# OpenDriveLab/OccNet

Hardware: AMD Instinct MI355X
Metric: nuScenes samples/sec (6-cam 900x1600 -> 200x200x16 voxels) (higher is better)
Workload: dtype f32 hot path (GEMM operands bf16x3-split, SCA value rows q16 block floating point) + bf16 backbone; 1 GPU; bevformer_base_occ forward: 6x(3x928x1600) images -> ResNet-50+FPN -> 4 BEVFormer layers (TSA+SCA+FFN) -> lifter + 2xConv3d decoder -> 200x200x16 voxels x (17 logits + 2 flow); history_frames=0, mode=infer, scope=e2e, input=resident-f32, samples_per_gpu=1, global_batch=1, parallelism=dp1, step_graph=False, linear_precision=bf16x3, backbone_dtype=bf16

## Files before the change

### include/occnet_amd.h

```cpp
#ifndef OCCNET_AMD_H_
#define OCCNET_AMD_H_

#include <stdint.h>

#ifdef __cplusplus
extern "C" {
#endif

#define OCC_OK 0
#define OCC_E_INVALID (-1)
#define OCC_E_LAUNCH (-2)
#define OCC_E_UNSUPPORTED (-3)

int occ_abi_version(void);
const char* occ_last_error(void);
int occ_selftest_fdiv_f32(const float* a, const float* d, float* q, int64_t n, void* stream);


int occ_ms_deform_attn_forward_f32(const float* value, const int64_t* spatial_shapes,
                                   const int64_t* level_start_index, const float* sampling_loc,
                                   const float* attn_weight, float* out, int B, int S, int M, int D,
                                   int L, int Lq, int P, int im2col_step, void* stream);

int occ_ms_deform_attn_backward_f32(const float* value, const int64_t* spatial_shapes,
// ... 120 lines not shown
                                     float* zv, int64_t ldzv, int M, void* stream);

int occ_sca_prep_forward_f32(const float* proj, int64_t proj_batch_stride, int proj_ld, const int64_t* row_to_query,
                             const float* ref_rb, const int64_t* spatial_shapes, float* loc, float* attn, int B,
                             int64_t R, int M, int L, int P, int Z, void* stream);
int occ_sca_prep_backward_f32(const float* grad_loc, const float* grad_attn, const float* attn,
                              const int64_t* query_to_rows, int Kq, const int64_t* spatial_shapes, float* dproj,
                              int proj_ld, int B, int64_t R, int64_t Q, int M, int L, int P, void* stream);

int occ_rows_gather_sum_f32(const float* x, int64_t x_batch_stride, const int64_t* index, int K, float* out, int B,
                            int64_t rows_out, int64_t rows_in, int F, void* stream);

int64_t occ_linear_wgrad_workspace_bytes(int M, int N, int K);
int occ_linear_wgrad_bf16x3_f32(const float* dy, int64_t lddy, const float* x, int64_t ldx, float* dw, float* db,
                                void* workspace, int64_t workspace_bytes, int M, int N, int K, void* stream);

int64_t occ_conv3d_wgrad_workspace_bytes(int B, int Z, int Y, int X, int Cin);
int occ_conv3d_wgrad_bf16x3_f32(const float* dy_pad, const float* x_pad, float* dw, void* workspace,
                                int64_t workspace_bytes, int B, int Z, int Y, int X, int Cin, void* stream);

int occ_bias_act_nhwc_bf16(void* x, const float* bias, const void* residual, int64_t rows, int C, int relu,
                           void* stream);

int64_t occ_bias_act_bwd_partial_floats(int64_t rows, int C);
int occ_bias_act_bwd_nhwc_bf16(const void* grad_y, const void* y, void* g, float* partial, float* bias_grad,
                               int64_t rows, int C, int relu, void* stream);

int occ_conv_bn_fold_fwd_f32(const float* weight, const float* gamma, const float* beta, const float* rstd,
                             const float* mean_rstd, float* w_folded, void* w_folded_bf16_nhwc, float* bias, int Cout,
                             int Cin, int KH, int KW, void* stream);
int occ_conv_bn_fold_bwd_f32(const void* grad_w_bf16, int64_t stride_o, int64_t stride_i, int64_t stride_h, int64_t stride_w,
                             const float* weight, const float* gamma, const float* rstd, const float* mean_rstd,
                             const float* grad_bias, float* grad_weight, float* grad_gamma, int Cout, int Cin, int KH, int KW,
                             void* stream);

unsigned occ_ln_dropout_hash(unsigned index, unsigned seed_lo, unsigned seed_hi);
int64_t occ_dropout_add_ln_bwd_partial_floats(int64_t rows, int C);
int occ_dropout_add_ln_fwd_f32(const float* x, const float* residual, const float* gamma, const float* beta, float eps,
                               float p_drop, uint64_t seed, float* z, float* y, float* stats, int64_t rows, int C,
                               void* stream);
int occ_dropout_add_ln_bwd_f32(const float* grad_y, const float* z, const float* stats, const float* gamma, float p_drop,
                               uint64_t seed, float* grad_x, float* grad_residual, float* partial, float* grad_gamma_beta,
                               int64_t rows, int C, void* stream);

int occ_value_proj_bf16_f32(int n_segments, const void* const* a, const int64_t* lda, const int64_t* rows,
                            const int64_t* rows_per_group, const int64_t* out_row0,
                            const float* const* group_bias, int bias_groups, const void* weight_packed,
                            float* out, int64_t ldo, int K, int N, int64_t out_group_rows, void* stream);
int occ_value_proj_bf16_f16pairs(int n_segments, const void* const* a, const int64_t* lda, const int64_t* rows,
                            const int64_t* rows_per_group, const int64_t* out_row0,
                            const float* const* group_bias, int bias_groups, const void* weight_packed,
                            void* out, int64_t ldo, int K, int N, int64_t out_group_rows, const float* out_scale,
                            void* stream);
int occ_value_proj_bf16_q16pairs(int n_segments, const void* const* a, const int64_t* lda, const int64_t* rows,
                            const int64_t* rows_per_group, const int64_t* out_row0,
                            const float* const* group_bias, int bias_groups, const void* weight_packed,
                            void* out, int64_t ldo, int K, int N, int64_t out_group_rows, const float* out_scale,
                            void* stream);

int occ_value_range_scale_bf16(int n_segments, const void* const* a, const int64_t* lda, const int64_t* rows, int K,
                               int n_planes, const float* row_l1, const float* bias_max, float* scale_out,
                               uint32_t* work, void* stream);
int occ_value_range_scale_from_amax(const uint32_t* amax8, int n_planes, const float* row_l1, const float* bias_max,
                                    float* scale_out, void* stream);

int occ_value_proj_bf16_planes(int n_segments, const void* const* a, const int64_t* lda, const int64_t* rows,
                               const int64_t* rows_per_group, const int64_t* out_row0,
                               const float* const* group_bias, int bias_groups, const void* weight_packed, void* out,
                               int out_f16, int64_t ldo, int K, int n_planes, int plane_cols, int64_t plane_stride,
                               int64_t out_group_rows, const float* out_scale, void* stream);

int occ_stem_conv7x7_pool_f32_bf16(const float* x, const void* weight_frag, const float* bias, void* out,
                                   int batch, int H, int W, void* stream);
int occ_stem_conv7x7_pool_u8_bf16(const uint8_t* x, const void* weight_frag, const float* bias, void* out,
                                  int batch, int Hs, int Ws, int H, int W, const float* mean,
                                  const float* std, int to_rgb, void* stream);

int occ_bias_relu_maxpool_nhwc_bf16(const void* y, const float* bias, void* out, int batch, int H, int W, int C,
                                    void* stream);

int occ_conv1x1_nhwc_bf16(const void* x, const void* weight, const float* bias, const void* residual,
                          void* out, int batch, int Hin, int Win, int Cin, int Cout, int stride, int relu,
                          int residual_upsample2, void* stream);

int occ_conv3x3_pack_weight_bf16(const float* weight, void* packed, int Cout, int Cin, void* stream);
int occ_conv3x3_nhwc_bf16(const void* x, const void* weight_packed, const float* bias, void* out, int batch,
                          int H, int W, int Cin, int Cout, int stride, int relu, void* stream);
int occ_conv3x3_nhwc_bf16_amax(const void* x, const void* weight_packed, const float* bias, void* out, int batch,
                               int H, int W, int Cin, int Cout, int stride, int relu, uint32_t* amax8, void* stream);
int occ_conv3x3_nhwc_bf16_variant(const void* x, const void* weight_packed, const float* bias, void* out, int batch,
                                  int H, int W, int Cin, int Cout, int stride, int relu, uint32_t* amax8, int variant,
                                  void* stream);

int occ_mfma_pack_b_frag_bf16(const float* weight, void* packed, int N, int K, void* stream);

int occ_bottleneck64_nhwc_bf16(const void* x, const void* w1_frag, const float* b1, const void* w2_frag,
                               const float* b2, const void* w3_frag, const float* b3, void* out, int batch,
                               int H, int W, int Cin, int downsample, void* stream);

#ifdef __cplusplus
}
#endif
#endif
```

### occnet_amd/csrc/conv1x1_nhwc_bf16.hip

```cpp
#include "common.h"

namespace occ {

typedef float f32x16 __attribute__((ext_vector_type(16)));
typedef __bf16 bf16x8 __attribute__((ext_vector_type(8)));


__device__ __forceinline__ float c1_bf16_to_f32(unsigned short h) { return __uint_as_float((unsigned)h << 16); }

template <int NT, int RT>
__global__ __launch_bounds__(256) void conv1x1_nhwc_bf16_kernel(
    const uint4* __restrict__ x, const uint4* __restrict__ w, const float* __restrict__ bias,
    const unsigned short* __restrict__ residual, unsigned short* __restrict__ out, long M, int N, int K,
    int Hin, int Win, int Hout, int Wout, int stride, int relu, int res_up) {
  constexpr int KC = 32, kCLD = KC * 2 + 16, PC = KC / 8;
  constexpr int BM = 32 * RT, BN = 128 * NT, WR = 32 * NT, OLD = BN + 4;
  constexpr int AP = BM * PC / 256;
  constexpr int A_BYTES = BM * kCLD;
  constexpr int STAGE_BYTES = 2 * A_BYTES, OUT_BYTES = 32 * OLD * 4;
  __shared__ __attribute__((aligned(16))) char lds[STAGE_BYTES > OUT_BYTES ? STAGE_BYTES : OUT_BYTES];
  const int tid = threadIdx.x, lane = tid & 63, wave = tid >> 6;
  const int vi = lane & 31, kb = lane >> 5;
  const long m0 = (long)blockIdx.x * BM;
  const int n0 = blockIdx.y * BN;
  const int KQ = K / 8;
  const int NT32 = N / 32;

  f32x16 acc[RT][NT];
#pragma unroll
  for (int rt = 0; rt < RT; ++rt)
#pragma unroll
    for (int t = 0; t < NT; ++t)
#pragma unroll
      for (int r = 0; r < 16; ++r) acc[rt][t][r] = 0.f;

  static_assert(AP >= 1 && AP <= 2 && NT <= 2, "staging register budget");
  long aofs[AP];
  int adst[AP];
#pragma unroll
  for (int ap = 0; ap < AP; ++ap) {
    const int j = tid + 256 * ap;
    const int row = j / PC, piece = j % PC;
    long m = m0 + row;
    if (m >= M) m = M - 1;
    long pix = m;
    if (stride != 1) {
      const long hw = (long)Hout * Wout;
      const long n = m / hw, rem = m % hw;
      const int yo = (int)(rem / Wout), xo = (int)(rem % Wout);
      pix = (n * Hin + (long)yo * stride) * Win + (long)xo * stride;
    }
    aofs[ap] = pix * KQ + piece;
    adst[ap] = row * kCLD + piece * 16;
  }
  const int nt0 = min((n0 + wave * WR) / 32, NT32 - 1), nt1 = min((n0 + wave * WR) / 32 + (NT - 1), NT32 - 1);
  const long wl0 = (long)nt0 * 64 + lane, wl1 = (long)nt1 * 64 + lane;
  uint4 va0_0, va1_0, va0_1, va1_1;
  uint4 wa0_0, wa1_0, wb0_0, wb1_0, wa0_1, wa1_1, wb0_1, wb1_1, wa0_2, wa1_2, wb0_2, wb1_2;
#define OCC_C1_ISSUE_A(S, K0)                                                                     \
  {                                                                                               \
    const long kq = (K0) / 8;                                                                     \
    va0_##S = x[aofs[0] + kq];                                                                    \
    if (AP > 1) va1_##S = x[aofs[AP > 1 ? 1 : 0] + kq];                                           \
  }
#define OCC_C1_ISSUE_W(S, K0)                                                                     \
  {                                                                                               \
    const long k0 = (long)((K0) / 16) * NT32 * 64, k1 = k0 + (long)NT32 * 64;                     \
    wa0_##S = w[k0 + wl0]; wb0_##S = w[k1 + wl0];                                                 \
    if (NT > 1) { wa1_##S = w[k0 + wl1]; wb1_##S = w[k1 + wl1]; }                                 \
  }
#define OCC_C1_STEP(SA, SW, SWN, BUF, K_NEXT)                                                     \
  {                                                                                               \
    char* sA = lds + (BUF) * A_BYTES;                                                             \
    *reinterpret_cast<uint4*>(sA + adst[0]) = va0_##SA;                                           \
    if (AP > 1) *reinterpret_cast<uint4*>(sA + adst[AP > 1 ? 1 : 0]) = va1_##SA;                  \
    __syncthreads();                 \
    OCC_C1_ISSUE_A(SA, K_NEXT)                                                                    \
    OCC_C1_ISSUE_W(SWN, K_NEXT)                                                                   \
    bf16x8 af[RT][2];                                                                             \
    _Pragma("unroll") for (int rt = 0; rt < RT; ++rt)                                             \
      _Pragma("unroll") for (int ks = 0; ks < 2; ++ks)                                            \
        af[rt][ks] = *reinterpret_cast<const bf16x8*>(sA + (rt * 32 + vi) * kCLD + ks * 32 + kb * 16); \
    _Pragma("unroll") for (int rt = 0; rt < RT; ++rt) {                                           \
      acc[rt][0] = __builtin_amdgcn_mfma_f32_32x32x16_bf16(af[rt][0], __builtin_bit_cast(bf16x8, wa0_##SW), acc[rt][0], 0, 0, 0); \
      if (NT > 1) acc[rt][NT - 1] = __builtin_amdgcn_mfma_f32_32x32x16_bf16(af[rt][0], __builtin_bit_cast(bf16x8, wa1_##SW), acc[rt][NT - 1], 0, 0, 0); \
    }                                                                                             \
    _Pragma("unroll") for (int rt = 0; rt < RT; ++rt) {                                           \
      acc[rt][0] = __builtin_amdgcn_mfma_f32_32x32x16_bf16(af[rt][1], __builtin_bit_cast(bf16x8, wb0_##SW), acc[rt][0], 0, 0, 0); \
      if (NT > 1) acc[rt][NT - 1] = __builtin_amdgcn_mfma_f32_32x32x16_bf16(af[rt][1], __builtin_bit_cast(bf16x8, wb1_##SW), acc[rt][NT - 1], 0, 0, 0); \
    }                                                                                             \
  }

  const int NCHK = K / KC;
  const int rot = (int)((blockIdx.x * 5u + blockIdx.y * 3u) % (unsigned)NCHK);
#define OCC_C1_K(CI) ((((CI) < NCHK ? (CI) : NCHK - 1) + rot) % NCHK * KC)
  OCC_C1_ISSUE_A(0, OCC_C1_K(0))
  OCC_C1_ISSUE_W(0, OCC_C1_K(0))
  OCC_C1_ISSUE_A(1, OCC_C1_K(1))
  OCC_C1_ISSUE_W(1, OCC_C1_K(1))
  for (int ci = 0; ci < NCHK; ci += 6) {
    OCC_C1_STEP(0, 0, 2, 0, OCC_C1_K(ci + 2))
    if (ci + 1 < NCHK) OCC_C1_STEP(1, 1, 0, 1, OCC_C1_K(ci + 3))
    if (ci + 2 < NCHK) OCC_C1_STEP(0, 2, 1, 0, OCC_C1_K(ci + 4))
    if (ci + 3 < NCHK) OCC_C1_STEP(1, 0, 2, 1, OCC_C1_K(ci + 5))
    if (ci + 4 < NCHK) OCC_C1_STEP(0, 1, 0, 0, OCC_C1_K(ci + 6))
    if (ci + 5 < NCHK) OCC_C1_STEP(1, 2, 1, 1, OCC_C1_K(ci + 7))
  }
#undef OCC_C1_K
#undef OCC_C1_STEP
#undef OCC_C1_ISSUE_A
#undef OCC_C1_ISSUE_W

  const int c = lane * 4;
  const bool col_live = c < BN && n0 + c < N;
  float4 bv = make_float4(0.f, 0.f, 0.f, 0.f);
  if (col_live) bv = *reinterpret_cast<const float4*>(bias + n0 + c);
  float* sO = reinterpret_cast<float*>(lds);
#pragma unroll
  for (int rt = 0; rt < RT; ++rt) {
    __syncthreads();
#pragma unroll
    for (int t = 0; t < NT; ++t)
#pragma unroll
      for (int r = 0; r < 16; ++r)
        sO[((r & 3) + 8 * (r >> 2) + 4 * kb) * OLD + (wave * NT + t) * 32 + vi] = acc[rt][t][r];
    __syncthreads();
    uint2 rv[8];
#pragma unroll
    for (int rr = 0; rr < 8; ++rr) {
      long m = m0 + rt * 32 + wave * 8 + rr;
      if (m >= M) m = M - 1;
      rv[rr] = make_uint2(0u, 0u);
      if (residual != nullptr && col_live) {
        long rrow = m;
        if (res_up) {
          const long hw = (long)Hout * Wout;
          const long n = m / hw, rem = m - n * hw;
          const int yo = (int)(rem / Wout), xo = (int)(rem - (long)yo * Wout);
          rrow = (n * (Hout >> 1) + (yo >> 1)) * (Wout >> 1) + (xo >> 1);
        }
        rv[rr] = *reinterpret_cast<const uint2*>(residual + rrow * N + n0 + c);
      }
    }
#pragma unroll
    for (int rr = 0; rr < 8; ++rr) {
      const int row = wave * 8 + rr;
      const long m = m0 + rt * 32 + row;
      if (m < M && col_live) {
        float4 v = *reinterpret_cast<const float4*>(sO + row * OLD + c);
        v.x += bv.x; v.y += bv.y; v.z += bv.z; v.w += bv.w;
        v.x += c1_bf16_to_f32((unsigned short)(rv[rr].x & 0xffffu));
        v.y += c1_bf16_to_f32((unsigned short)(rv[rr].x >> 16));
        v.z += c1_bf16_to_f32((unsigned short)(rv[rr].y & 0xffffu));
        v.w += c1_bf16_to_f32((unsigned short)(rv[rr].y >> 16));
        if (relu) {
          v.x = fmaxf(v.x, 0.f); v.y = fmaxf(v.y, 0.f); v.z = fmaxf(v.z, 0.f); v.w = fmaxf(v.w, 0.f);
        }
        const uint2 o = make_uint2(pack_bf16x2_rne(v.x, v.y), pack_bf16x2_rne(v.z, v.w));
        *reinterpret_cast<uint2*>(out + m * N + n0 + c) = o;
      }
    }
  }
}

}

extern "C" int occ_conv1x1_nhwc_bf16(const void* x, const void* weight, const float* bias,
                                     const void* residual, void* out, int batch, int Hin, int Win,
                                     int Cin, int Cout, int stride, int relu, int residual_upsample2,
                                     void* stream) {
  using namespace occ;
  OCC_CHECK_ARG(x && weight && bias && out, "conv1x1_nhwc_bf16: null pointer argument");
  OCC_CHECK_ARG(batch > 0 && Hin > 0 && Win > 0 && Cin > 0 && Cout > 0 && stride > 0,
                "conv1x1_nhwc_bf16: bad dimension");
  if (Cin % 32 || Cout % 32) {
    set_error("conv1x1_nhwc_bf16: no kernel for Cin=%d Cout=%d (need Cin %% 32 == 0, Cout %% 32 == 0)", Cin,
              Cout);
    return OCC_E_UNSUPPORTED;
  }
  const int Hout = (Hin - 1) / stride + 1, Wout = (Win - 1) / stride + 1;
  OCC_CHECK_ARG(!residual_upsample2 || (residual && Hout % 2 == 0 && Wout % 2 == 0),
                "conv1x1_nhwc_bf16: an upsampled residual needs even output sizes (exact x2 nearest upsampling)");
  const long M = (long)batch * Hout * Wout;
  hipStream_t st = reinterpret_cast<hipStream_t>(stream);
#define OCC_C1_LAUNCH(NTT, RTT, BNN)                                                                \
  hipLaunchKernelGGL((conv1x1_nhwc_bf16_kernel<NTT, RTT>),                                          \
                     dim3((unsigned)((M + 32 * RTT - 1) / (32 * RTT)), (unsigned)((Cout + BNN - 1) / BNN)), \
                     dim3(256), 0, st, reinterpret_cast<const uint4*>(x),                           \
                     reinterpret_cast<const uint4*>(weight), bias,                                  \
                     reinterpret_cast<const unsigned short*>(residual),                             \
                     reinterpret_cast<unsigned short*>(out), M, Cout, Cin, Hin, Win, Hout, Wout, stride, relu,  \
                     residual_upsample2)
  if (Cout <= 128) OCC_C1_LAUNCH(1, 2, 128); else OCC_C1_LAUNCH(2, 2, 256);
#undef OCC_C1_LAUNCH
  OCC_CHECK_LAUNCH("conv1x1_nhwc_bf16");
  return OCC_OK;
}
```

### occnet_amd/ext.py

```python
import ctypes
import os

import torch

from . import _lib, cache_epoch
from ._lib import OccAmdError, OccAmdUnsupported, f32, i32, i64, ptr, stream_ptr


_TIMING = None
_TIMING_ONLY = None


def kernel_timing(enable=True):
    global _TIMING, _TIMING_ONLY
    _TIMING = {} if enable else None
    _TIMING_ONLY = None
    return _TIMING


def kernel_timing_only(names):
    global _TIMING_ONLY
    _TIMING_ONLY = None if names is None else set(names)


# ... 1330 lines not shown
    so, si, sh, sw = grad_w16.stride()
    with torch.cuda.device(weight.device):
        rc = _lib.lib().occ_conv_bn_fold_bwd_f32(ptr(grad_w16), i64(so), i64(si), i64(sh), i64(sw), ptr(weight), ptr(gamma),
                                                 ptr(rstd), ptr(mean_rstd), ptr(grad_bias), ptr(dW), ptr(dgamma), i32(O), i32(I),
                                                 i32(KH), i32(KW), stream_ptr(weight.device))
    _lib.check(rc, "conv_bn_fold_bwd")
    return dW, dgamma


def stem_pack_weight(weight):
    if tuple(weight.shape) != (64, 3, 7, 7):
        raise OccAmdUnsupported("stem_pack_weight: expected a (64, 3, 7, 7) weight")
    w2 = torch.zeros(64, 7, 8, 4, dtype=torch.float32, device=weight.device)
    w2[:, :, :7, :3] = weight.float().permute(0, 2, 3, 1)
    return mfma_pack_b_frag(w2.reshape(64, 224))


def stem_conv7x7_pool(x, weight_frag, bias):
    _need_cuda_f32("x", x)
    _need_cuda_f32("bias", bias)
    if x.dim() != 4 or x.shape[1] != 3 or not x.is_contiguous():
        raise OccAmdUnsupported("stem_conv7x7_pool: x must be a contiguous (N, 3, H, W) fp32 tensor")
    if weight_frag.numel() != 64 * 224 or bias.numel() != 64:
        raise OccAmdError("stem_conv7x7_pool: inconsistent shapes")
    N, _, H, W = x.shape
    Hc, Wc = (H - 1) // 2 + 1, (W - 1) // 2 + 1
    Hp, Wp = (Hc - 1) // 2 + 1, (Wc - 1) // 2 + 1
    out = torch.empty((N, 64, Hp, Wp), dtype=torch.bfloat16, device=x.device, memory_format=torch.channels_last)
    with torch.cuda.device(x.device), _timed('bb_stem7x7_pool'):
        rc = _lib.lib().occ_stem_conv7x7_pool_f32_bf16(ptr(x), ptr(weight_frag), ptr(bias), ptr(out), i32(N),
                                                       i32(H), i32(W), stream_ptr(x.device))
    _note_flops('bb_stem7x7_pool', 2.0 * N * Hc * Wc * 64 * 147)
    _lib.check(rc, "stem_conv7x7_pool")
    return out


def stem_conv7x7_pool_u8(x_u8, weight_frag, bias, mean, std, to_rgb=False, size_divisor=32):
    if not (x_u8.is_cuda and x_u8.dtype == torch.uint8 and x_u8.dim() == 4 and x_u8.shape[-1] == 3
            and x_u8.is_contiguous()):
        raise OccAmdUnsupported("stem_conv7x7_pool_u8: x must be a contiguous (N, H, W, 3) uint8 device tensor")
    _need_cuda_f32("bias", bias)
    if weight_frag.numel() != 64 * 224 or bias.numel() != 64:
        raise OccAmdError("stem_conv7x7_pool_u8: inconsistent shapes")
    N, Hs, Ws, _ = x_u8.shape
    d = int(size_divisor)
    H, W = (Hs + d - 1) // d * d, (Ws + d - 1) // d * d
    Hc, Wc = (H - 1) // 2 + 1, (W - 1) // 2 + 1
    Hp, Wp = (Hc - 1) // 2 + 1, (Wc - 1) // 2 + 1
    out = torch.empty((N, 64, Hp, Wp), dtype=torch.bfloat16, device=x_u8.device, memory_format=torch.channels_last)
    mean_c = (f32 * 3)(*[float(v) for v in mean])
    std_c = (f32 * 3)(*[float(v) for v in std])
    with torch.cuda.device(x_u8.device):
        rc = _lib.lib().occ_stem_conv7x7_pool_u8_bf16(ptr(x_u8), ptr(weight_frag), ptr(bias), ptr(out), i32(N),
                                                      i32(Hs), i32(Ws), i32(H), i32(W), mean_c, std_c,
                                                      i32(1 if to_rgb else 0), stream_ptr(x_u8.device))
    _lib.check(rc, "stem_conv7x7_pool_u8")
    return out, (H, W)


def bias_relu_maxpool_nhwc(y, bias):
    if not (y.is_cuda and y.dtype == torch.bfloat16 and y.dim() == 4
            and y.is_contiguous(memory_format=torch.channels_last)):
        raise OccAmdUnsupported("bias_relu_maxpool_nhwc: y must be a channels_last bfloat16 device tensor")
    _need_cuda_f32("bias", bias)
    N, C, H, W = y.shape
    if bias.numel() != C:
        raise OccAmdError("bias_relu_maxpool_nhwc: bias must have C entries")
    out = torch.empty((N, C, (H - 1) // 2 + 1, (W - 1) // 2 + 1), dtype=torch.bfloat16, device=y.device,
                      memory_format=torch.channels_last)
    with torch.cuda.device(y.device):
        rc = _lib.lib().occ_bias_relu_maxpool_nhwc_bf16(ptr(y), ptr(bias), ptr(out), i32(N), i32(H), i32(W),
                                                        i32(C), stream_ptr(y.device))
    _lib.check(rc, "bias_relu_maxpool_nhwc")
    return out


def conv1x1_pack_weight(weight2d):
    cout, cin = weight2d.shape
    if cin % 32 or cout % 32:
        raise OccAmdUnsupported("conv1x1_pack_weight: Cin and Cout must be multiples of 32")
    return mfma_pack_b_frag(weight2d.float().contiguous())


def conv1x1_nhwc(x, weight_frag, bias, residual=None, relu=False, stride=1, residual_upsample2=False):
    if not (x.is_cuda and x.dtype == torch.bfloat16 and x.dim() == 4
            and x.is_contiguous(memory_format=torch.channels_last)):
        raise OccAmdUnsupported("conv1x1_nhwc: x must be a channels_last bfloat16 device tensor")
    _need_cuda_f32("bias", bias)
    N, Cin, H, W = x.shape
    Cout = bias.numel()
    if not (weight_frag.dtype == torch.int16 and weight_frag.dim() == 1 and weight_frag.is_contiguous()
            and weight_frag.numel() == Cout * Cin):
        raise OccAmdError("conv1x1_nhwc: weight must come from conv1x1_pack_weight (Cout*Cin bf16, fragment order)")
    s = int(stride)
    Ho, Wo = (H - 1) // s + 1, (W - 1) // s + 1
    out = torch.empty((N, Cout, Ho, Wo), dtype=torch.bfloat16, device=x.device,
                      memory_format=torch.channels_last)
    want = (N, Cout, Ho // 2, Wo // 2) if residual_upsample2 else tuple(out.shape)
    if residual_upsample2 and (residual is None or Ho % 2 or Wo % 2):
        raise OccAmdUnsupported("conv1x1_nhwc: an upsampled residual needs even output sizes")
    if residual is not None and not (residual.dtype == torch.bfloat16 and tuple(residual.shape) == want and
                                     residual.is_contiguous(memory_format=torch.channels_last)):
        raise OccAmdUnsupported("conv1x1_nhwc: residual must match the output (channels_last bfloat16)")
    with torch.cuda.device(x.device), _timed('bb_conv1x1'):
        rc = _lib.lib().occ_conv1x1_nhwc_bf16(ptr(x), ptr(weight_frag), ptr(bias), ptr(residual), ptr(out),
                                              i32(N), i32(H), i32(W), i32(Cin), i32(Cout), i32(s),
                                              i32(1 if relu else 0), i32(1 if residual_upsample2 else 0),
                                              stream_ptr(x.device))
    _note_flops('bb_conv1x1', 2.0 * N * Ho * Wo * Cin * Cout)
    _lib.check(rc, "conv1x1_nhwc")
    return out


def mfma_pack_b_frag(weight2d):
    _need_cuda_f32("weight", weight2d)
    if weight2d.dim() != 2:
        raise OccAmdError("mfma_pack_b_frag: expected a (N, K) matrix")
    weight2d = weight2d.contiguous()
    n, k = weight2d.shape
    packed = torch.empty(n * k, dtype=torch.int16, device=weight2d.device)
    with torch.cuda.device(weight2d.device):
        rc = _lib.lib().occ_mfma_pack_b_frag_bf16(ptr(weight2d), ptr(packed), i32(n), i32(k),
                                                  stream_ptr(weight2d.device))
    _lib.check(rc, "mfma_pack_b_frag")
    return packed


def bottleneck64_pack(w1, b1, w2, b2, w3, b3, wds=None, bds=None):
    w1 = w1.float().reshape(w1.shape[0], -1)
    w3 = w3.float().reshape(w3.shape[0], -1)
    if tuple(w2.shape) != (64, 64, 3, 3) or w1.shape[0] != 64 or tuple(w3.shape) != (256, 64):
        raise OccAmdUnsupported("bottleneck64_pack: only 64 mid / 256 output channels")
    ds = wds is not None
    cin = w1.shape[1]
    if (ds and cin != 64) or (not ds and cin != 256):
        raise OccAmdUnsupported("bottleneck64_pack: Cin must be 256 (identity) or 64 (projection)")
    w2m = w2.float().permute(0, 2, 3, 1).reshape(64, 9 * 64)
    b3 = b3.float()
    if ds:
        w3 = torch.cat([w3, wds.float().reshape(256, 64)], dim=1)
        b3 = b3 + bds.float()
    return dict(w1=mfma_pack_b_frag(w1), b1=b1.float().contiguous(), w2=mfma_pack_b_frag(w2m),
                b2=b2.float().contiguous(), w3=mfma_pack_b_frag(w3), b3=b3.contiguous(), cin=cin, ds=ds)


def bottleneck64_nhwc(x, pack):
    if not (x.is_cuda and x.dtype == torch.bfloat16 and x.dim() == 4
            and x.is_contiguous(memory_format=torch.channels_last)):
        raise OccAmdUnsupported("bottleneck64_nhwc: x must be a channels_last bfloat16 device tensor")
    N, Cin, H, W = x.shape
    if Cin != pack['cin']:
        raise OccAmdError("bottleneck64_nhwc: x has %d channels, the pack was built for %d" % (Cin, pack['cin']))
    out = torch.empty((N, 256, H, W), dtype=torch.bfloat16, device=x.device, memory_format=torch.channels_last)
    with torch.cuda.device(x.device), _timed('bb_bottleneck64'):
        rc = _lib.lib().occ_bottleneck64_nhwc_bf16(ptr(x), ptr(pack['w1']), ptr(pack['b1']), ptr(pack['w2']),
                                                   ptr(pack['b2']), ptr(pack['w3']), ptr(pack['b3']), ptr(out),
                                                   i32(N), i32(H), i32(W), i32(Cin), i32(1 if pack['ds'] else 0),
                                                   stream_ptr(x.device))
    _note_flops('bb_bottleneck64', 2.0 * N * H * W * (Cin * 64 + 9 * 64 * 64 + 64 * 256 + (Cin * 256 if pack['ds'] else 0)))
    _lib.check(rc, "bottleneck64_nhwc")
    return out


def conv3x3_pack_weight(weight):
    _need_cuda_f32("weight", weight)
    if weight.dim() != 4 or tuple(weight.shape[2:]) != (3, 3):
        raise OccAmdError("conv3x3_pack_weight: expected a (Cout, Cin, 3, 3) weight")
    cout, cin = weight.shape[:2]
    packed = torch.empty(weight.numel(), dtype=torch.int16, device=weight.device)
    with torch.cuda.device(weight.device):
        rc = _lib.lib().occ_conv3x3_pack_weight_bf16(ptr(weight), ptr(packed), i32(cout), i32(cin),
                                                     stream_ptr(weight.device))
    _lib.check(rc, "conv3x3_pack_weight")
    return packed


def conv3x3_nhwc(x, w_packed, bias, cout, relu=False, stride=1, amax=None, variant=None):
    if not (x.is_cuda and x.dtype == torch.bfloat16 and x.dim() == 4
            and x.is_contiguous(memory_format=torch.channels_last)):
        raise OccAmdUnsupported("conv3x3_nhwc: x must be a channels_last bfloat16 device tensor")
    _need_cuda_f32("bias", bias)
    N, Cin, H, W = x.shape
    if w_packed.numel() != cout * Cin * 9 or bias.numel() != cout:
        raise OccAmdError("conv3x3_nhwc: inconsistent shapes")
    st = int(stride)
    if st not in (1, 2):
        raise OccAmdUnsupported("conv3x3_nhwc: stride must be 1 or 2")
    if amax is not None and not (amax.is_cuda and amax.dtype == torch.int32 and amax.numel() == 8 and amax.is_contiguous()):
        raise OccAmdError("conv3x3_nhwc: amax must be 8 contiguous int32 device words")
    out = torch.empty((N, cout, (H - 1) // st + 1, (W - 1) // st + 1), dtype=torch.bfloat16, device=x.device,
                      memory_format=torch.channels_last)
# ... 18 lines not shown
```

### tools_dev/conv_probe.py

```python
import os, sys
sys.path.insert(0, os.path.join(os.path.dirname(os.path.abspath(__file__)), ".."))
import torch
from occnet_amd import ext


def timeit(fn, iters=20):
    for _ in range(3):
        fn()
    a, b = torch.cuda.Event(enable_timing=True), torch.cuda.Event(enable_timing=True)
    torch.cuda.synchronize(); a.record()
    for _ in range(iters):
        fn()
    b.record(); torch.cuda.synchronize()
    return a.elapsed_time(b) * 1e3 / iters


def main(which):
    g = torch.Generator().manual_seed(0)
    N = 6
    mk = lambda *s: (torch.randn(*s, generator=g) * 0.05).cuda()
    act = lambda c, h, w: torch.randn(N, c, h, w, generator=g).cuda().to(torch.bfloat16).contiguous(
        memory_format=torch.channels_last)
    if 'c3' in which or 'c3v' in which:
        def variants(s, cout):
            if 'c3v' not in which:
                return (None,)
            vs = (12, 13, 14, 16, 18, 22, 23, 24) if s == 1 else (12, 13, 22)
            return (None,) + tuple(v for v in vs if cout % (128 * (v // 10)) == 0)
        for (cin, cout, h, w, s) in [(128, 128, 232, 400, 2), (128, 128, 116, 200, 1), (256, 256, 116, 200, 2),
                                     (256, 256, 58, 100, 1), (512, 512, 58, 100, 2), (512, 512, 29, 50, 1),
                                     (256, 256, 116, 200, 1), (256, 256, 29, 50, 1),
                                     (256, 256, 29, 50, 2)]:
            x, wp, b = act(cin, h, w), ext.conv3x3_pack_weight(mk(cout, cin, 3, 3)), mk(cout)
            vs = variants(s, cout)
            rounds = 5 if len(vs) > 1 else 1
            times = {v: [] for v in vs}
            for _ in range(rounds):
                for v in vs:
                    times[v].append(timeit(lambda: ext.conv3x3_nhwc(x, wp, b, cout, relu=True, stride=s, variant=v)))
            for v in vs:
                us = sorted(times[v])[rounds // 2]
                ho, wo = (h - 1) // s + 1, (w - 1) // s + 1
                fl = 2.0 * N * ho * wo * cout * cin * 9
                tag = 'auto' if v is None else f'v{v}'
                print(f"conv3x3 {cin:4d}->{cout:4d} {h:3d}x{w:3d} s{s} {tag:4s}: {us:7.1f} us  {fl / us * 1e-6:6.1f} TF/s")
    if 'c1' in which:
        for (cin, cout, h, w, s, res) in [(256, 128, 232, 400, 1, 0), (128, 512, 116, 200, 1, 1),
                                          (512, 128, 116, 200, 1, 0), (256, 512, 232, 400, 2, 0),
                                          (512, 256, 116, 200, 1, 0), (256, 1024, 58, 100, 1, 1),
                                          (1024, 256, 58, 100, 1, 0), (512, 1024, 116, 200, 2, 0),
                                          (1024, 512, 58, 100, 1, 0), (512, 2048, 29, 50, 1, 1),
                                          (2048, 512, 29, 50, 1, 0), (1024, 2048, 58, 100, 2, 0),
                                          (512, 256, 116, 200, 1, 0), (1024, 256, 58, 100, 1, 0),
                                          (2048, 256, 29, 50, 1, 0)]:
            x, wp, b = act(cin, h, w), ext.conv1x1_pack_weight(mk(cout, cin)), mk(cout)
            ho, wo = (h - 1) // s + 1, (w - 1) // s + 1
            r = act(cout, ho, wo) if res else None
            us = timeit(lambda: ext.conv1x1_nhwc(x, wp, b, residual=r, relu=True, stride=s))
            fl = 2.0 * N * ho * wo * cout * cin
            mb = N * (ho * wo * (cin + cout * (2 if res else 1))) * 2 / 1e6
            print(f"conv1x1 {cin:4d}->{cout:4d} {h:3d}x{w:3d} s{s} res{res}: {us:7.1f} us  {fl / us * 1e-6:6.1f} TF/s  "
                  f"{mb / us:5.2f} TB/s")


def vp():
    g = torch.Generator().manual_seed(0)
    w = (torch.randn(256, 256, generator=g) / 16).cuda()
    gb = torch.randn(6, 256, generator=g).cuda()
    total = 23200 + 5800 + 1450 + 375
    out = torch.empty(6 * total, 256, device='cuda')
    hws = (23200, 5800, 1450, 375)
    a_list = [torch.randn(6 * hw, 256, generator=g).cuda().to(torch.bfloat16) for hw in hws]
    gb4 = gb.unsqueeze(0).repeat(4, 1, 1).contiguous()
    starts = [0, 23200, 29000, 30450]
    us = timeit(lambda: ext.value_proj_bf16(a_list, w, gb4, out, rows_per_group=list(hws), out_group_rows=total,
                                            out_row0=starts))
    mb = 6 * total * 256 * (2 + 4) / 1e6
    print(f"value_proj_bf16 all levels M={6 * total}: {us:7.1f} us  {mb / us:5.2f} TB/s")
    x = torch.randn(6 * total, 256, generator=g).cuda()
    b = torch.randn(256, generator=g).cuda()
    us = timeit(lambda: ext.linear(x, w, b))
    print(f"linear bf16x3 f32 in M={6 * total}: {us:7.1f} us")


if __name__ == '__main__':
    if 'vp' in sys.argv[1:]:
        vp()
    main(sys.argv[1:] or ['c3', 'c1'])
```

Baseline: 190.2 samples/s.

## Add split-K and tile-size variants to conv1x1 NHWC kernel with per-shape pick table

```diff
diff --git a/include/occnet_amd.h b/include/occnet_amd.h
--- a/include/occnet_amd.h
+++ b/include/occnet_amd.h
@@ -226,6 +226,11 @@
 int occ_conv1x1_nhwc_bf16(const void* x, const void* weight, const float* bias, const void* residual,
                           void* out, int batch, int Hin, int Win, int Cin, int Cout, int stride, int relu,
                           int residual_upsample2, void* stream);
+int occ_conv1x1_nhwc_bf16_variant(const void* x, const void* weight, const float* bias, const void* residual,
+                                  void* out, int batch, int Hin, int Win, int Cin, int Cout, int stride, int relu,
+                                  int residual_upsample2, int variant, void* workspace, int64_t workspace_bytes,
+                                  void* stream);
+int64_t occ_conv1x1_nhwc_bf16_workspace_bytes(int batch, int Hin, int Win, int Cin, int Cout, int stride, int variant);
 
 int occ_conv3x3_pack_weight_bf16(const float* weight, void* packed, int Cout, int Cin, void* stream);
 int occ_conv3x3_nhwc_bf16(const void* x, const void* weight_packed, const float* bias, void* out, int batch,
diff --git a/occnet_amd/csrc/conv1x1_nhwc_bf16.hip b/occnet_amd/csrc/conv1x1_nhwc_bf16.hip
--- a/occnet_amd/csrc/conv1x1_nhwc_bf16.hip
+++ b/occnet_amd/csrc/conv1x1_nhwc_bf16.hip
@@ -12,7 +12,8 @@
 __global__ __launch_bounds__(256) void conv1x1_nhwc_bf16_kernel(
     const uint4* __restrict__ x, const uint4* __restrict__ w, const float* __restrict__ bias,
     const unsigned short* __restrict__ residual, unsigned short* __restrict__ out, long M, int N, int K,
-    int Hin, int Win, int Hout, int Wout, int stride, int relu, int res_up) {
+    int Hin, int Win, int Hout, int Wout, int stride, int relu, int res_up, float* __restrict__ slabs,
+    unsigned* __restrict__ tile_cnt) {
   constexpr int KC = 32, kCLD = KC * 2 + 16, PC = KC / 8;
   constexpr int BM = 32 * RT, BN = 128 * NT, WR = 32 * NT, OLD = BN + 4;
   constexpr int AP = BM * PC / 256;
@@ -91,9 +92,11 @@
     }                                                                                             \
   }
 
-  const int NCHK = K / KC;
+  const int nslice = (int)gridDim.z, slice = (int)blockIdx.z;
+  const int c_lo = (int)((long)slice * (K / KC) / nslice);
+  const int NCHK = (int)((long)(slice + 1) * (K / KC) / nslice) - c_lo;
   const int rot = (int)((blockIdx.x * 5u + blockIdx.y * 3u) % (unsigned)NCHK);
-#define OCC_C1_K(CI) ((((CI) < NCHK ? (CI) : NCHK - 1) + rot) % NCHK * KC)
+#define OCC_C1_K(CI) (((((CI) < NCHK ? (CI) : NCHK - 1) + rot) % NCHK + c_lo) * KC)
   OCC_C1_ISSUE_A(0, OCC_C1_K(0))
   OCC_C1_ISSUE_W(0, OCC_C1_K(0))
   OCC_C1_ISSUE_A(1, OCC_C1_K(1))
@@ -110,6 +113,53 @@
 #undef OCC_C1_STEP
 #undef OCC_C1_ISSUE_A
 #undef OCC_C1_ISSUE_W
+
+  if (nslice > 1) {
+    constexpr int TILE_G = BM * BN / 2;
+    const long tile = (long)blockIdx.y * gridDim.x + blockIdx.x;
+    unsigned long long* tslab = reinterpret_cast<unsigned long long*>(slabs) + tile * nslice * TILE_G;
+#pragma unroll
+    for (int rt = 0; rt < RT; ++rt)
+#pragma unroll
+      for (int t = 0; t < NT; ++t)
+#pragma unroll
+        for (int q = 0; q < 8; ++q) {
+          const unsigned long long g = ((unsigned long long)__float_as_uint(acc[rt][t][2 * q + 1]) << 32) |
+                                       __float_as_uint(acc[rt][t][2 * q]);
+          __hip_atomic_store(tslab + (long)slice * TILE_G + (((rt * NT + t) * 4 + wave) * 8 + q) * 64 + lane, g,
+                             __ATOMIC_RELAXED, __HIP_MEMORY_SCOPE_AGENT);
+        }
+    asm volatile("s_waitcnt vmcnt(0)" ::: "memory");
+    __syncthreads();
+    int* last_flag = reinterpret_cast<int*>(lds);
+    if (tid == 0) {
+      const unsigned prev = __hip_atomic_fetch_add(tile_cnt + tile, 1u, __ATOMIC_RELAXED, __HIP_MEMORY_SCOPE_AGENT);
+      *last_flag = prev == (unsigned)(nslice - 1);
+    }
+    __syncthreads();
+    if (!*last_flag) return;
+#pragma unroll
+    for (int rt = 0; rt < RT; ++rt)
+#pragma unroll
+      for (int t = 0; t < NT; ++t) {
+        f32x16 sum;
+        for (int sl = 0; sl < nslice; ++sl) {
+          f32x16 v = acc[rt][t];
+          if (sl != slice) {
+            unsigned long long* src = tslab + (long)sl * TILE_G + (((rt * NT + t) * 4 + wave) * 8) * 64 + lane;
+#pragma unroll
+            for (int q = 0; q < 8; ++q) {
+              const unsigned long long g = __hip_atomic_load(src + q * 64, __ATOMIC_RELAXED, __HIP_MEMORY_SCOPE_AGENT);
+              v[2 * q] = __uint_as_float((unsigned)g);
+              v[2 * q + 1] = __uint_as_float((unsigned)(g >> 32));
+            }
+          }
+          if (sl == 0) sum = v;
+          else sum += v;
+        }
+        acc[rt][t] = sum;
+      }
+  }
 
   const int c = lane * 4;
   const bool col_live = c < BN && n0 + c < N;
@@ -163,12 +213,41 @@
   }
 }
 
-}
-
-extern "C" int occ_conv1x1_nhwc_bf16(const void* x, const void* weight, const float* bias,
-                                     const void* residual, void* out, int batch, int Hin, int Win,
-                                     int Cin, int Cout, int stride, int relu, int residual_upsample2,
-                                     void* stream) {
+
+__global__ __launch_bounds__(256) void conv1x1_clear_counters_kernel(unsigned* __restrict__ cnt, int n) {
+  for (int i = blockIdx.x * 256 + threadIdx.x; i < n; i += gridDim.x * 256)
+    __hip_atomic_store(cnt + i, 0u, __ATOMIC_RELAXED, __HIP_MEMORY_SCOPE_AGENT);
+}
+
+bool c1_variant_known(int id) {
+  const int s = id / 100, nt = id / 10 % 10, rt = id % 10;
+  return id > 0 && (s == 0 || s == 2 || s == 4 || s == 8) && (nt == 1 || nt == 2) && (rt == 2 || rt == 4);
+}
+int c1_slices(int id) { return id >= 100 ? id / 100 : 1; }
+
+struct C1Pick { long M; int K, N, stride, id; };
+constexpr C1Pick kC1Picks[] = {
+    {556800, 256, 128, 1, 14},
+};
+
+int c1_pick(long M, int K, int N, int stride, bool allow_split) {
+  for (const C1Pick& p : kC1Picks)
+    if (p.M == M && p.K == K && p.N == N && p.stride == stride && (allow_split || p.id < 100)) return p.id;
+  return N <= 128 ? 12 : 22;
+}
+
+long long c1_workspace_bytes(long M, int N, int id) {
+  const int s = c1_slices(id), nt = id / 10 % 10, rt = id % 10;
+  if (s == 1) return 0;
+  const long long tiles = ((M + 32 * rt - 1) / (32 * rt)) * (long long)((N + 128 * nt - 1) / (128 * nt));
+  return tiles * s * (32LL * rt) * (128LL * nt) * 4 + (tiles * 4 + 255) / 256 * 256;
+}
+}
+
+static int conv1x1_nhwc_bf16_launch(const void* x, const void* weight, const float* bias, const void* residual,
+                                    void* out, int batch, int Hin, int Win, int Cin, int Cout, int stride, int relu,
+                                    int residual_upsample2, int variant, bool allow_split, void* workspace,
+                                    long long workspace_bytes, void* stream) {
   using namespace occ;
   OCC_CHECK_ARG(x && weight && bias && out, "conv1x1_nhwc_bf16: null pointer argument");
   OCC_CHECK_ARG(batch > 0 && Hin > 0 && Win > 0 && Cin > 0 && Cout > 0 && stride > 0,
@@ -182,17 +261,79 @@
   OCC_CHECK_ARG(!residual_upsample2 || (residual && Hout % 2 == 0 && Wout % 2 == 0),
                 "conv1x1_nhwc_bf16: an upsampled residual needs even output sizes (exact x2 nearest upsampling)");
   const long M = (long)batch * Hout * Wout;
+  const int id = variant == 0 ? c1_pick(M, Cin, Cout, stride, allow_split) : variant;
+  const int S = c1_slices(id);
+  if (!c1_variant_known(id) || S > Cin / 32) {
+    set_error("conv1x1_nhwc_bf16: no variant %d for Cin %d (100 * S + 10 * NT + RT: S 1, 2, 4, 8 with S <= Cin / 32, "
+              "NT 1, 2, RT 2, 4)", variant, Cin);
+    return OCC_E_UNSUPPORTED;
+  }
+  const long long need = c1_workspace_bytes(M, Cout, id);
+  if (need > 0 && (workspace == nullptr || workspace_bytes < need)) {
+    set_error("conv1x1_nhwc_bf16: variant %d needs a workspace of %lld bytes (given %lld)", id, need,
+              workspace ? workspace_bytes : 0LL);
+    return OCC_E_INVALID;
+  }
   hipStream_t st = reinterpret_cast<hipStream_t>(stream);
-#define OCC_C1_LAUNCH(NTT, RTT, BNN)                                                                \
-  hipLaunchKernelGGL((conv1x1_nhwc_bf16_kernel<NTT, RTT>),                                          \
-                     dim3((unsigned)((M + 32 * RTT - 1) / (32 * RTT)), (unsigned)((Cout + BNN - 1) / BNN)), \
-                     dim3(256), 0, st, reinterpret_cast<const uint4*>(x),                           \
-                     reinterpret_cast<const uint4*>(weight), bias,                                  \
+  const int nt = id / 10 % 10, rt = id % 10;
+  const unsigned gx = (unsigned)((M + 32 * rt - 1) / (32 * rt)), gy = (unsigned)((Cout + 128 * nt - 1) / (128 * nt));
+  float* slabs = nullptr;
+  unsigned* cnt = nullptr;
+  if (S > 1) {
+    slabs = reinterpret_cast<float*>(workspace);
+    cnt = reinterpret_cast<unsigned*>(reinterpret_cast<char*>(workspace) + (long long)gx * gy * S * (32 * rt) *
+                                      (128 * nt) * 4);
+    const int n = (int)(gx * gy);
+    hipLaunchKernelGGL(conv1x1_clear_counters_kernel, dim3((unsigned)min((n + 255) / 256, 64)), dim3(256), 0, st, cnt, n);
+    OCC_CHECK_LAUNCH("conv1x1_nhwc_bf16 (split-K counters)");
+  }
+#define OCC_C1_LAUNCH(NTT, RTT)                                                                     \
+  hipLaunchKernelGGL((conv1x1_nhwc_bf16_kernel<NTT, RTT>), dim3(gx, gy, (unsigned)S), dim3(256), 0, st, \
+                     reinterpret_cast<const uint4*>(x), reinterpret_cast<const uint4*>(weight), bias, \
                      reinterpret_cast<const unsigned short*>(residual),                             \
                      reinterpret_cast<unsigned short*>(out), M, Cout, Cin, Hin, Win, Hout, Wout, stride, relu,  \
-                     residual_upsample2)
-  if (Cout <= 128) OCC_C1_LAUNCH(1, 2, 128); else OCC_C1_LAUNCH(2, 2, 256);
+                     residual_upsample2, slabs, cnt)
+  switch (id % 100) {
+    case 12: OCC_C1_LAUNCH(1, 2); break;
+    case 14: OCC_C1_LAUNCH(1, 4); break;
+    case 22: OCC_C1_LAUNCH(2, 2); break;
+    default: OCC_C1_LAUNCH(2, 4); break;
+  }
 #undef OCC_C1_LAUNCH
   OCC_CHECK_LAUNCH("conv1x1_nhwc_bf16");
   return OCC_OK;
 }
+
+extern "C" int occ_conv1x1_nhwc_bf16(const void* x, const void* weight, const float* bias,
+                                     const void* residual, void* out, int batch, int Hin, int Win,
+                                     int Cin, int Cout, int stride, int relu, int residual_upsample2,
+                                     void* stream) {
+  return conv1x1_nhwc_bf16_launch(x, weight, bias, residual, out, batch, Hin, Win, Cin, Cout, stride, relu,
+                                  residual_upsample2, 0, false, nullptr, 0, stream);
+}
+
+extern "C" int occ_conv1x1_nhwc_bf16_variant(const void* x, const void* weight, const float* bias,
+                                             const void* residual, void* out, int batch, int Hin, int Win, int Cin,
+                                             int Cout, int stride, int relu, int residual_upsample2, int variant,
+                                             void* workspace, int64_t workspace_bytes, void* stream) {
+  return conv1x1_nhwc_bf16_launch(x, weight, bias, residual, out, batch, Hin, Win, Cin, Cout, stride, relu,
+                                  residual_upsample2, variant, true, workspace, workspace_bytes, stream);
+}
+
+extern "C" int64_t occ_conv1x1_nhwc_bf16_workspace_bytes(int batch, int Hin, int Win, int Cin, int Cout, int stride,
+                                                         int variant) {
+  using namespace occ;
+  OCC_CHECK_ARG(batch > 0 && Hin > 0 && Win > 0 && Cin > 0 && Cout > 0 && stride > 0,
+                "conv1x1_nhwc_bf16_workspace_bytes: bad dimension");
+  if (Cin % 32 || Cout % 32) {
+    set_error("conv1x1_nhwc_bf16_workspace_bytes: no kernel for Cin=%d Cout=%d", Cin, Cout);
+    return OCC_E_UNSUPPORTED;
+  }
+  const long M = (long)batch * ((Hin - 1) / stride + 1) * ((Win - 1) / stride + 1);
+  const int id = variant == 0 ? c1_pick(M, Cin, Cout, stride, true) : variant;
+  if (!c1_variant_known(id) || c1_slices(id) > Cin / 32) {
+    set_error("conv1x1_nhwc_bf16_workspace_bytes: no variant %d for Cin %d", variant, Cin);
+    return OCC_E_UNSUPPORTED;
+  }
+  return c1_workspace_bytes(M, Cout, id);
+}
diff --git a/occnet_amd/ext.py b/occnet_amd/ext.py
--- a/occnet_amd/ext.py
+++ b/occnet_amd/ext.py
@@ -1436,7 +1436,23 @@
     return mfma_pack_b_frag(weight2d.float().contiguous())
 
 
-def conv1x1_nhwc(x, weight_frag, bias, residual=None, relu=False, stride=1, residual_upsample2=False):
+_C1_WS = {}
+
+
+def conv1x1_workspace_bytes(N, H, W, cin, cout, stride=1, variant=0):
+    key = (N, H, W, cin, cout, stride, variant)
+    nbytes = _C1_WS.get(key)
+    if nbytes is None:
+        lib = _lib.lib()
+        lib.occ_conv1x1_nhwc_bf16_workspace_bytes.restype = ctypes.c_int64
+        nbytes = int(lib.occ_conv1x1_nhwc_bf16_workspace_bytes(i32(N), i32(H), i32(W), i32(cin), i32(cout),
+                                                                 i32(stride), i32(variant)))
+        _lib.check(min(nbytes, 0), "conv1x1_workspace_bytes")
+        _C1_WS[key] = nbytes
+    return nbytes
+
+
+def conv1x1_nhwc(x, weight_frag, bias, residual=None, relu=False, stride=1, residual_upsample2=False, variant=None):
     if not (x.is_cuda and x.dtype == torch.bfloat16 and x.dim() == 4
             and x.is_contiguous(memory_format=torch.channels_last)):
         raise OccAmdUnsupported("conv1x1_nhwc: x must be a channels_last bfloat16 device tensor")
@@ -1456,11 +1472,14 @@
     if residual is not None and not (residual.dtype == torch.bfloat16 and tuple(residual.shape) == want and
                                      residual.is_contiguous(memory_format=torch.channels_last)):
         raise OccAmdUnsupported("conv1x1_nhwc: residual must match the output (channels_last bfloat16)")
+    v = 0 if variant is None else int(variant)
     with torch.cuda.device(x.device), _timed('bb_conv1x1'):
-        rc = _lib.lib().occ_conv1x1_nhwc_bf16(ptr(x), ptr(weight_frag), ptr(bias), ptr(residual), ptr(out),
-                                              i32(N), i32(H), i32(W), i32(Cin), i32(Cout), i32(s),
-                                              i32(1 if relu else 0), i32(1 if residual_upsample2 else 0),
-                                              stream_ptr(x.device))
+        nbytes = conv1x1_workspace_bytes(N, H, W, Cin, Cout, s, v)
+        ws = torch.empty(nbytes, dtype=torch.uint8, device=x.device) if nbytes > 0 else None
+        rc = _lib.lib().occ_conv1x1_nhwc_bf16_variant(ptr(x), ptr(weight_frag), ptr(bias), ptr(residual), ptr(out),
+                                                      i32(N), i32(H), i32(W), i32(Cin), i32(Cout), i32(s),
+                                                      i32(1 if relu else 0), i32(1 if residual_upsample2 else 0),
+                                                      i32(v), ptr(ws), i64(nbytes), stream_ptr(x.device))
     _note_flops('bb_conv1x1', 2.0 * N * Ho * Wo * Cin * Cout)
     _lib.check(rc, "conv1x1_nhwc")
     return out
diff --git a/tools_dev/conv1x1_launch_table.py b/tools_dev/conv1x1_launch_table.py
--- /dev/null
+++ b/tools_dev/conv1x1_launch_table.py
@@ -0,0 +1,67 @@
+#!/usr/bin/env python
+import re
+import statistics
+import sys
+
+B = 6
+STEP = ([("L2 b0 ds", 232, 400, 256, 512, 2, 0), ("L2 b0 conv1", 232, 400, 256, 128, 1, 0),
+         ("L2 b0 conv3", 116, 200, 128, 512, 1, 1)] +
+        [(f"L2 b{i} {c}", 116, 200, ci, co, 1, r) for i in (1, 2, 3)
+         for c, ci, co, r in (("conv1", 512, 128, 0), ("conv3", 128, 512, 1))] +
+        [("L3 b0 ds", 116, 200, 512, 1024, 2, 0), ("L3 b0 conv1", 116, 200, 512, 256, 1, 0),
+         ("L3 b0 conv3", 58, 100, 256, 1024, 1, 1)] +
+        [(f"L3 b{i} {c}", 58, 100, ci, co, 1, r) for i in range(1, 6)
+         for c, ci, co, r in (("conv1", 1024, 256, 0), ("conv3", 256, 1024, 1))] +
+        [("L4 b0 ds", 58, 100, 1024, 2048, 2, 0), ("L4 b0 conv1", 58, 100, 1024, 512, 1, 0),
+         ("L4 b0 conv3", 29, 50, 512, 2048, 1, 1)] +
+        [(f"L4 b{i} {c}", 29, 50, ci, co, 1, r) for i in (1, 2)
+         for c, ci, co, r in (("conv1", 2048, 512, 0), ("conv3", 512, 2048, 1))] +
+        [("FPN lat L4", 29, 50, 2048, 256, 1, 0), ("FPN lat L3 +up2", 58, 100, 1024, 256, 1, 2),
+         ("FPN lat L2 +up2", 116, 200, 512, 256, 1, 2)])
+assert len(STEP) == 32
+
+
+def shape_m(sh):
+    _, h, w, _, _, s, _ = sh
+    return B * ((h - 1) // s + 1) * ((w - 1) // s + 1)
+
+
+def floor_us(sh):
+    _, h, w, cin, cout, s, res = sh
+    m = shape_m(sh)
+    nbytes = 2 * (B * h * w * cin / (s * s) + m * cout + (m * cout / (4 if res == 2 else 1) if res else 0))
+    return max(nbytes / 6.3e6, 2.0 * m * cin * cout / 2.5e9)
+
+
+def fits(row, sh):
+    m, cout = shape_m(sh), sh[4]
+    return any(row[1] == (m + 32 * rt - 1) // (32 * rt) and row[2] == (cout + 128 * nt - 1) // (128 * nt)
+               for nt in (1, 2) for rt in (2, 4))
+
+
+def main(path):
+    rows = []
+    for line in open(path):
+        m = re.match(r"\s*([\d.]+) us\s+grid \((\d+), (\d+)\)\s+(.*)", line)
+        if m:
+            rows.append((float(m.group(1)), int(m.group(2)) // 256, int(m.group(3)), m.group(4)))
+    steps = [rows[i:i + len(STEP)] for i in range(len(rows) - len(STEP) + 1)
+             if all(fits(r, sh) for r, sh in zip(rows[i:i + len(STEP)], STEP))]
+    if not steps:
+        sys.exit("no inference step (32 matching conv1x1 launches) in the dump")
+    print(f"# {len(steps)} inference steps; median per launch position; floor = max(bytes / 6.3 TB/s, FLOP / 2.5 PF)")
+    print(f"{'launch':18s} {'M x K -> N':>22s} {'blocks':>12s} {'floor':>6s} {'us':>7s}  kernel")
+    tot = ftot = 0.0
+    for i, sh in enumerate(STEP):
+        us = statistics.median(s[i][0] for s in steps)
+        fl = floor_us(sh)
+        tot += us
+        ftot += fl
+        k = re.sub(r"\(.*", "", steps[-1][i][3]).replace("void occ::", "")
+        mkn = f"{shape_m(sh)} x {sh[3]} -> {sh[4]}" + (" s2" if sh[5] == 2 else "")
+        print(f"{sh[0]:18s} {mkn:>22s} {steps[-1][i][1]:>6d} x {steps[-1][i][2]:<3d} {fl:6.1f} {us:7.1f}  {k}")
+    print(f"{'total per step':18s} {'':>22s} {'':>12s} {ftot:6.1f} {tot:7.1f}")
+
+
+if __name__ == '__main__':
+    main(sys.argv[1])
diff --git a/tools_dev/conv_probe.py b/tools_dev/conv_probe.py
--- a/tools_dev/conv_probe.py
+++ b/tools_dev/conv_probe.py
@@ -13,6 +13,16 @@
         fn()
     b.record(); torch.cuda.synchronize()
     return a.elapsed_time(b) * 1e3 / iters
+
+
+C1_STEP_SHAPES = [("L2 b0 conv1", 256, 128, 232, 400, 1, 0), ("L2 ds", 256, 512, 232, 400, 2, 0),
+                  ("L2 conv3", 128, 512, 116, 200, 1, 1), ("L2 conv1", 512, 128, 116, 200, 1, 0),
+                  ("L3 b0 conv1", 512, 256, 116, 200, 1, 0), ("FPN lat L2", 512, 256, 116, 200, 1, 2),
+                  ("L3 ds", 512, 1024, 116, 200, 2, 0), ("L3 conv3", 256, 1024, 58, 100, 1, 1),
+                  ("L3 conv1", 1024, 256, 58, 100, 1, 0), ("FPN lat L3", 1024, 256, 58, 100, 1, 2),
+                  ("L4 b0 conv1", 1024, 512, 58, 100, 1, 0), ("L4 ds", 1024, 2048, 58, 100, 2, 0),
+                  ("L4 conv3", 512, 2048, 29, 50, 1, 1), ("L4 conv1", 2048, 512, 29, 50, 1, 0),
+                  ("FPN lat L4", 2048, 256, 29, 50, 1, 0)]
 
 
 def main(which):
@@ -44,6 +54,29 @@
                 fl = 2.0 * N * ho * wo * cout * cin * 9
                 tag = 'auto' if v is None else f'v{v}'
                 print(f"conv3x3 {cin:4d}->{cout:4d} {h:3d}x{w:3d} s{s} {tag:4s}: {us:7.1f} us  {fl / us * 1e-6:6.1f} TF/s")
+    if any(a.startswith('c1v') for a in which):
+        sel = [a for a in which if a.startswith('c1v=')]
+        rows = [int(i) for i in sel[0][4:].split(',')] if sel else range(len(C1_STEP_SHAPES))
+        for i in rows:
+            name, cin, cout, h, w, s, res = C1_STEP_SHAPES[i]
+            ho, wo = (h - 1) // s + 1, (w - 1) // s + 1
+            x, wp, b = act(cin, h, w), ext.conv1x1_pack_weight(mk(cout, cin)), mk(cout)
+            r = act(cout, ho // 2, wo // 2) if res == 2 else (act(cout, ho, wo) if res else None)
+            vs = [None] + [sl * 100 + v for sl in (0, 2, 4, 8) for v in (12, 14, 22, 24) if sl <= cin // 32]
+            times = {v: [] for v in vs}
+            for _ in range(5):
+                for v in vs:
+                    times[v].append(timeit(lambda: ext.conv1x1_nhwc(x, wp, b, residual=r, relu=res != 2, stride=s,
+                                                                    residual_upsample2=res == 2, variant=v)))
+            fl = 2.0 * N * ho * wo * cout * cin
+            mb = N * (h * w * cin / (s * s) + ho * wo * cout + (ho * wo * cout / (4 if res == 2 else 1) if res else 0)) \
+                * 2 / 1e6
+            floor = max(mb / 6.3, fl / 2.5e9)
+            for v in vs:
+                us = sorted(times[v])[2]
+                tag = 'auto' if v is None else f'v{v}'
+                print(f"c1 {i:2d} {name:18s} {cin:4d}->{cout:4d} {h:3d}x{w:3d} s{s} res{res} {tag:5s}: {us:7.1f} us  "
+                      f"floor {floor:5.1f}  {fl / us * 1e-6:6.1f} TF/s  {mb / us:5.2f} TB/s", flush=True)
     if 'c1' in which:
         for (cin, cout, h, w, s, res) in [(256, 128, 232, 400, 1, 0), (128, 512, 116, 200, 1, 1),
                                           (512, 128, 116, 200, 1, 0), (256, 512, 232, 400, 2, 0),
```

Result: no change. 191.0 samples/s (median of 6 runs) (+0.4%).
